# baldhat/yolov10-3D

Measured on AMD Instinct MI355X. Metric: train_images_per_sec, higher is better.
Workload: dtype bf16

## Files before the change

### yolov10-3d_amd/csrc/conv_gemm.hip

```cpp
#include "common.h"
#include "conv_frag.h"
#include <cstdlib>

namespace {

struct ConvP {
  const void* x;
  const void* w;
  const float* bias;
  const float* scale;
  const float* shift;
  int act;
  void* y;
  float* part;
  long xsb, xsh, xsw;
  long ysw;
  int B, Hg, Wg;
  int Hq, Wq;
  int Cg, Cn, G;
  int kh, kw, stride, pad;
  int Ktot, Kpad;
  int M;
  int ntx, nty;
};
// ... 531 lines not shown
  long n = (long)Cout * Kpad;
  if (idx >= n) return;
  int k = idx % Kpad;
  int co = idx / Kpad;
  float v = 0.f;
  if (k < taps * Cg_pad) {
    int tap = k / Cg_pad, ci = k - tap * Cg_pad;
    if (ci < Cg) v = w[((long)co * Cg + ci) * taps + tap];
  }
  TT<T>::st(out + idx, v);
}

template <typename T>
__global__ void pack_w_dgrad_kernel(const float* __restrict__ w, T* __restrict__ out, int G, int Cn, int Cg, int taps, int Kpad) {
  long idx = (long)blockIdx.x * blockDim.x + threadIdx.x;
  long n = (long)G * Cg * Kpad;
  if (idx >= n) return;
  int k = idx % Kpad;
  int ci = (idx / Kpad) % Cg;
  int g = idx / ((long)Kpad * Cg);
  float v = 0.f;
  if (k < taps * Cn) {
    int tap = k / Cn, co = k - tap * Cn;
    v = w[((long)(g * Cn + co) * Cg + ci) * taps + tap];
  }
  TT<T>::st(out + idx, v);
}

template <typename T>
__global__ __launch_bounds__(256) void mt_pack_w_kernel(const long* __restrict__ desc, const int* __restrict__ ctensor, const int* __restrict__ coff,
                                                        int chunk) {
  constexpr int CAP = 4096;
  __shared__ float st[CAP + 64];
  const long* d = desc + (long)ctensor[blockIdx.x] * 8;
  const float* __restrict__ w = (const float*)d[0];
  T* __restrict__ out = (T*)d[1];
  const int a = (int)d[2], b = (int)d[3], c = (int)d[4], taps = (int)d[5], Kpad = (int)d[6], mode = (int)d[7];
  const long n = mode == 0 ? (long)a * Kpad : (long)a * c * Kpad;
  const long beg = (long)coff[blockIdx.x] * chunk;
  const long end = beg + chunk < n ? beg + chunk : n;
  const int tid = threadIdx.x;
  const long rb = beg / Kpad, re = (end - 1) / Kpad;
  if (mode == 0) {
    for (long idx = beg + tid; idx < end; idx += 256) {
      const int k = (int)(idx % Kpad), co = (int)(idx / Kpad);
      float v = 0.f;
      if (k < taps * c) {
        const int tap = k / c, ci = k - tap * c;
        if (ci < b) v = w[((long)co * b + ci) * taps + tap];
      }
      TT<T>::st(out + idx, v);
    }
  } else {
    const int CB = b < 256 ? b : 256;
    int R = CAP / (taps * (CB + 1));
    if (R < 1) R = 1;
    const int P = CB + 1;
    for (long r0 = rb; r0 <= re;) {
      const int g = (int)(r0 / c), ci0 = (int)(r0 - (long)g * c);
      int nr = R;
      if (nr > c - ci0) nr = c - ci0;
      if (nr > re - r0 + 1) nr = (int)(re - r0 + 1);
      const int seg = nr * taps;
      for (int co0 = 0; co0 < b; co0 += CB) {
        const int cb = b - co0 < CB ? b - co0 : CB;
        __syncthreads();
        for (int i = tid; i < cb * seg; i += 256) {
          const int col = i / seg, j = i - col * seg;
          st[j * P + col] = w[((long)(g * b + co0 + col) * c + ci0) * taps + j];
        }
        __syncthreads();
        for (int o = tid; o < seg * cb; o += 256) {
          const int j = o / cb, col = o - j * cb;
          const int cil = j / taps, tap = j - cil * taps;
          const long idx = (r0 + cil) * Kpad + (long)tap * b + co0 + col;
          if (idx >= beg && idx < end) TT<T>::st(out + idx, st[j * P + col]);
        }
      }
      for (int o = tid; o < nr * (Kpad - taps * b); o += 256) {
        const int rl = o / (Kpad - taps * b), k = taps * b + o - rl * (Kpad - taps * b);
        const long idx = (r0 + rl) * Kpad + k;
        if (idx >= beg && idx < end) TT<T>::st(out + idx, 0.f);
      }
      r0 += nr;
    }
  }
}

template <typename T, int MODE>
int launch_conv_mode(ConvP p, hipStream_t st) {
  dim3 block(256);
  const unsigned ny = MODE == 2 ? 4 : 1;
  p.ntx = MODE == 2 ? cdiv((long)p.B * ((p.Hq + 1) / 2) * ((p.Wq + 1) / 2), 128) : cdiv(p.M, 128);
  const long t128 = (long)p.ntx * cdiv(p.Cn, 128) * ny * p.G;
  int bc = p.Cn > 64 ? 128 : (p.Cn > 32 ? 64 : 32);
  if (p.Cn % 32 == 0) {
    if (bc == 128 && t128 < 192) bc = 64;
    if (bc == 64 && (long)p.ntx * cdiv(p.Cn, 64) * ny * p.G < 192 && p.Cn > 32) bc = 32;
  }
  p.nty = cdiv(p.Cn, bc);
  if (bc == 128) {
    size_t sm = 2 * (128 + 128) * 128;
    hipLaunchKernelGGL((conv_gemm_kernel<T, 128, 128, 2, 2, MODE>), dim3(p.ntx * p.nty, ny, p.G), block, sm, st, p);
  } else if (bc == 64) {
    size_t sm = 2 * (128 + 64) * 128;
    hipLaunchKernelGGL((conv_gemm_kernel<T, 128, 64, 4, 1, MODE>), dim3(p.ntx * p.nty, ny, p.G), block, sm, st, p);
  } else {
    size_t sm = 2 * (128 + 32) * 128;
    hipLaunchKernelGGL((conv_gemm_kernel<T, 128, 32, 4, 1, MODE>), dim3(p.ntx * p.nty, ny, p.G), block, sm, st, p);
  }
  Y3D_LAUNCH_CHECK();
  return Y3D_OK;
}

template <typename T, bool DGRAD>
int launch_conv(ConvP p, hipStream_t st) {
  if (DGRAD && p.kh == 3 && p.kw == 3 && p.stride == 2 && p.pad == 1 && p.Cg % TT<T>::CE == 0) return launch_conv_mode<T, 2>(p, st);
  return launch_conv_mode<T, DGRAD ? 1 : 0>(p, st);
}

}

int y3d_conv3x3_tile_route(int dtype, int B, int H, int W, int Cg, int Cn, int G, int kh, int kw, int stride, int pad);
int y3d_conv3x3_flat_tiles(int B, int H, int W);
int y3d_conv3x3_tile_launch(int dtype, int route, const void* x, long xsb, long xsh, long xsw, int B, int H, int W, int Cg, int Cn, int G,
                            const void* w, int Ktot, void* y, long ysw, float* part, int flip, const float* scale, const float* shift, int act,
                            void* stream);

int y3d_wgrad_tile_height(int dtype, int H, int W, int Cg, int Cn, int kh, int kw, int stride, int pad);
int y3d_wgrad_tile_splits(int th, int B, int H, int W, int Cg, int Cn, int G);
int y3d_conv3x3_wgrad_tile_launch(int th, const void* x, long xsb, long xsh, long xsw, const void* dy, long dsw, int B, int H, int W, int Cg,
                                  int Cn, int G, float* slab, int nsplit, void* stream);

int y3d_conv1x1_stream_ok(int dtype, long M, int K, int N, long xsw, int G = 1);
int y3d_conv1x1_stream_launch(const void* x, long xsw, const void* w, int Kpad, const float* bias, const float* scale, const float* shift, int act,
                              void* y, long ysw, float* part, long M, int K, int N, int G, void* stream);
int y3d_wgrad1x1_stream_ok(int dtype, long M, int Cg, int Cn, long xsw, long dsw);
int y3d_wgrad1x1_stream_launch(const void* x, long xsw, const void* dy, long dsw, long M, int Cg, int Cn, float* slab, int nsplit, int chunk_px,
                               void* stream);
int y3d_conv3x3s2_dgrad_ok(int dtype, int B, int Ho, int Wo, int H, int W, int Cout, int Cin, long dsw, long xsw);
int y3d_conv3x3s2_dgrad_launch(const void* dy, long dsw, int B, int Ho, int Wo, int Cout, const void* w_packed_dgrad, int Kpad, void* dx, long xsw,
                               int H, int W, int Cin, void* stream);
int y3d_conv3x3_small_ok(int dtype, int B, int H, int W, int Cin, int Cout, int rows);
int y3d_conv3x3_small_launch(const void* x, long xsb, long xsh, long xsw, int B, int H, int W, int Cin, int Cout, const void* w, int Ktot, void* y,
                             long ysw, float* part, int rows, int flip, const float* scale, const float* shift, int act, const void* res, long rsw,
                             void* stream);
int y3d_conv3x3_small_rows(int B, int H, int W, int Cin, int Cout);
int y3d_conv3x3_small_s2_ok(int dtype, int B, int H, int W, int Cin, int Cout);
int y3d_conv3x3_small_s2_rows(int B, int H, int W, int Cin, int Cout);
int y3d_conv3x3_small_s2_launch(const void* x, long xsb, long xsh, long xsw, int B, int H, int W, int Cin, int Cout, const void* w, int Ktot, void* y,
                                long ysw, float* part, int rows, const float* scale, const float* shift, int act, void* stream);
int y3d_conv1x1_stream_rows(long M, int K, int N, int G = 1);
int y3d_wgrad3x3_small_ok(int dtype, int B, int H, int W, int Cin, int Cout);
int y3d_wgrad3x3_small_splits(int B, int H, int W);
int y3d_wgrad3x3_small_launch(const void* x, long xsb, long xsh, long xsw, const void* dy, long dsw, int B, int H, int W, int Cin, int Cout,
                              float* slab, int nsplit, void* stream);
static inline bool dense_pixels(int B, int H, int W, long sb, long sh, long sw) {
  return (H == 1 || sh == (long)W * sw) && (B == 1 || sb == (long)H * W * sw);
}

static int g_tile_kernels = 1;
extern "C" int y3d_conv2d_wgrad_splits(int dtype, int B, int Ho, int Wo, int Cout, int Cin_g, int groups, int kh, int kw);

static int conv_route(int dtype, int op, int epi, int B, int H, int W, int Ho, int Wo, int Cin, int Cout, int groups, int kh, int kw, int stride,
                      int pad, bool dense, long asw, long bsw, bool cin_full) {
  const int ce = dtype == Y3D_BF16 ? 8 : 4;
  const bool k1 = kh == 1 && kw == 1 && stride == 1 && pad == 0, k3s1 = kh == 3 && kw == 3 && stride == 1 && pad == 1,
             k3s2 = kh == 3 && kw == 3 && stride == 2 && pad == 1;
  if (op == Y3D_OP_FWD) {
    Y3D_CHECK(dtype == Y3D_BF16 || dtype == Y3D_F32, "conv2d_fwd: bad dtype %d", dtype);
    Y3D_CHECK(B > 0 && H > 0 && W > 0 && Cin > 0 && Cout > 0 && groups > 0, "conv2d_fwd: empty shape");
    Y3D_CHECK(Cin % groups == 0 && Cout % groups == 0, "conv2d_fwd: channels not divisible by groups");
    Y3D_CHECK((Cin / groups) % ce == 0, "conv2d_fwd: Cin/groups=%d must be a multiple of %d (pad the input)", Cin / groups, ce);
    Y3D_CHECK(kh * kw <= 64, "conv2d_fwd: at most 64 filter taps");
    Y3D_CHECK(epi >= Y3D_EPI_RAW && epi <= Y3D_EPI_BIAS, "conv2d_fwd: bad epilogue %d", epi);
    const int Cg = Cin / groups, Cn = Cout / groups;
    const long M = (long)B * Ho * Wo;
    const bool bias = epi == Y3D_EPI_BIAS;
    if (k1 && dense && y3d_conv1x1_stream_ok(dtype, M, Cg, Cn, asw, groups)) return Y3D_ROUTE_STREAM1X1;
    Y3D_CHECK(!(epi == Y3D_EPI_PARTIALS && k1 && y3d_conv1x1_stream_ok(dtype, M, Cg, Cn, Cin, groups)),
              "conv2d_fwd: 1x1 input view must be pixel-dense and below 4 GB for the BatchNorm partial layout of this shape");
    if (k3s1 && groups == 1 && !bias && y3d_conv3x3_small_ok(dtype, B, H, W, Cin, Cout, 1)) return Y3D_ROUTE_SMALL;
    Y3D_CHECK(epi != Y3D_EPI_AFFINE_RES, "conv2d_fwd_affine_res: no kernel with a residual epilogue takes this geometry (ask y3d_conv2d_fwd_affine_res_ok first)");
    if (k3s2 && groups == 1 && !bias && y3d_conv3x3_small_s2_ok(dtype, B, H, W, Cin, Cout)) return Y3D_ROUTE_SMALL_S2;
    if (!bias && g_tile_kernels) return y3d_conv3x3_tile_route(dtype, B, H, W, Cg, Cn, groups, kh, kw, stride, pad);
    return Y3D_ROUTE_GENERIC;
  }
  if (op == Y3D_OP_BWD_DATA) {
    Y3D_CHECK(dtype == Y3D_BF16 || dtype == Y3D_F32, "conv2d_bwd_data: bad dtype %d", dtype);
    Y3D_CHECK(groups > 0 && Cin % groups == 0 && Cout % groups == 0, "conv2d_bwd_data: channels not divisible by groups");
    Y3D_CHECK((Cout / groups) % ce == 0, "conv2d_bwd_data: Cout/groups=%d must be a multiple of %d", Cout / groups, ce);
    Y3D_CHECK(kh * kw <= 64, "conv2d_bwd_data: at most 64 filter taps");
    Y3D_CHECK(epi == 0, "conv2d_bwd_data: no epilogue variants");
    const int Cg = Cout / groups, Cn = Cin / groups;
    if (k1 && dense && y3d_conv1x1_stream_ok(dtype, (long)B * H * W, Cg, Cn, asw, groups)) return Y3D_ROUTE_STREAM1X1;
    if (k3s1 && groups == 1 && Ho == H && Wo == W && y3d_conv3x3_small_ok(dtype, B, H, W, Cout, Cin, 1)) return Y3D_ROUTE_SMALL;
    if (k3s2 && groups == 1 && dense && y3d_conv3x3s2_dgrad_ok(dtype, B, Ho, Wo, H, W, Cout, Cin, asw, bsw)) return Y3D_ROUTE_S2_DGRAD;
    if (g_tile_kernels && Ho == H && Wo == W) return y3d_conv3x3_tile_route(dtype, B, H, W, Cg, Cn, groups, kh, kw, stride, pad);
    return Y3D_ROUTE_GENERIC;
  }
  Y3D_CHECK(op == Y3D_OP_BWD_WEIGHT, "conv2d_route: bad op %d", op);
  Y3D_CHECK(dtype == Y3D_BF16 || dtype == Y3D_F32, "conv2d_bwd_weight: bad dtype %d", dtype);
  Y3D_CHECK(groups > 0 && Cin % groups == 0 && Cout % groups == 0, "conv2d_bwd_weight: channels not divisible by groups");
  Y3D_CHECK((Cin / groups) % ce == 0 && (Cout / groups) % ce == 0, "conv2d_bwd_weight: per-group channels must be multiples of %d", ce);
  Y3D_CHECK(epi == 0, "conv2d_bwd_weight: no epilogue variants");
  if (k3s1 && groups == 1 && cin_full && y3d_wgrad3x3_small_ok(dtype, B, H, W, Cin, Cout)) return Y3D_ROUTE_WGRAD_SMALL;
  if (g_tile_kernels && cin_full && y3d_wgrad_tile_height(dtype, H, W, Cin / groups, Cout / groups, kh, kw, stride, pad)) return Y3D_ROUTE_WGRAD_TILE;
  if (k1 && groups == 1 && cin_full && dense && y3d_wgrad1x1_stream_ok(dtype, (long)B * Ho * Wo, Cin, Cout, asw, bsw)) return Y3D_ROUTE_WGRAD_STREAM1X1;
  return Y3D_ROUTE_GENERIC;
}

extern "C" {

int y3d_get_tile_kernels(void) { return g_tile_kernels; }

int y3d_set_tile_kernels(int enable) {
  int old = g_tile_kernels;
  g_tile_kernels = enable ? 1 : 0;
  return old;
}

int y3d_conv_stat_blocks(int B, int Ho, int Wo) { return cdiv((long)B * Ho * Wo, 128); }

int y3d_conv2d_route(int dtype, int op, int epi, int B, int H, int W, int Cin, int Cout, int groups, int kh, int kw, int stride, int pad) {
  Y3D_CHECK(kh > 0 && kw > 0 && stride > 0 && pad >= 0, "conv2d_route: bad filter geometry");
  const int Ho = (H + 2 * pad - kh) / stride + 1, Wo = (W + 2 * pad - kw) / stride + 1;
  Y3D_CHECK(Ho > 0 && Wo > 0, "conv2d_route: empty output");
  if (op == Y3D_OP_BWD_DATA) return conv_route(dtype, op, epi, B, H, W, Ho, Wo, Cin, Cout, groups, kh, kw, stride, pad, true, Cout, Cin, true);
  return conv_route(dtype, op, epi, B, H, W, Ho, Wo, Cin, Cout, groups, kh, kw, stride, pad, true, Cin, Cout, true);
}

int y3d_conv2d_wgrad_plan(int dtype, int B, int H, int W, int Cin, int Cout, int groups, int kh, int kw, int stride, int pad) {
  int Ho = (H + 2 * pad - kh) / stride + 1, Wo = (W + 2 * pad - kw) / stride + 1;
  switch (conv_route(dtype, Y3D_OP_BWD_WEIGHT, 0, B, H, W, Ho, Wo, Cin, Cout, groups, kh, kw, stride, pad, true, Cin, Cout, true)) {
    case Y3D_ROUTE_WGRAD_SMALL: return y3d_wgrad3x3_small_splits(B, H, W);
    case Y3D_ROUTE_WGRAD_TILE:
      return y3d_wgrad_tile_splits(y3d_wgrad_tile_height(dtype, H, W, Cin / groups, Cout / groups, kh, kw, stride, pad), B, H, W, Cin / groups,
                                   Cout / groups, groups);
    case Y3D_ROUTE_WGRAD_STREAM1X1: {
      const int target = 256;
      const long tiles = (long)cdiv(Cin, Cin <= 64 ? 64 : 128) * cdiv(Cout, Cout <= 64 ? 64 : 128);
      long want = target / tiles, maxs = cdiv((long)B * H * W, 4 * 64);
      if (want > maxs) want = maxs;
      return (int)(want < 1 ? 1 : want);
    }
    default: return y3d_conv2d_wgrad_splits(dtype, B, Ho, Wo, Cout, Cin / groups, groups, kh, kw);
  }
}

int y3d_conv2d_stat_rows(int dtype, int B, int H, int W, int Cin, int Cout, int groups, int kh, int kw, int stride, int pad) {
  int Ho = (H + 2 * pad - kh) / stride + 1, Wo = (W + 2 * pad - kw) / stride + 1;
  switch (conv_route(dtype, Y3D_OP_FWD, Y3D_EPI_PARTIALS, B, H, W, Ho, Wo, Cin, Cout, groups, kh, kw, stride, pad, true, Cin, Cout, true)) {
    case Y3D_ROUTE_STREAM1X1: return y3d_conv1x1_stream_rows((long)B * H * W, Cin / groups, Cout / groups, groups);
    case Y3D_ROUTE_SMALL: return y3d_conv3x3_small_rows(B, H, W, Cin, Cout);
    case Y3D_ROUTE_SMALL_S2: return y3d_conv3x3_small_s2_rows(B, H, W, Cin, Cout);
    case Y3D_ROUTE_FLAT: return y3d_conv3x3_flat_tiles(B, H, W);
    case Y3D_ROUTE_TILE8: case Y3D_ROUTE_WIDE3_8: return B * cdiv(H, 8) * cdiv(W, 16);
    case Y3D_ROUTE_TILE16: case Y3D_ROUTE_WIDE3_16: return B * cdiv(H, 16) * cdiv(W, 16);
    default: return cdiv((long)B * Ho * Wo, 128);
  }
}

int y3d_conv_kpad(int dtype, int k_total) {
  int ce = dtype == Y3D_BF16 ? 8 : 4;
  return cdiv(k_total, ce) * ce;
}

int y3d_pack_weight_fwd(int dtype, const float* w_oihw, void* out, int Cout, int Cin_g, int Cin_g_pad, int kh, int kw, void* stream) {
  int ce = dtype == Y3D_BF16 ? 8 : 4;
  Y3D_CHECK(Cin_g_pad >= Cin_g && Cin_g_pad % ce == 0, "pack_weight_fwd: Cin_g_pad=%d must be a multiple of %d", Cin_g_pad, ce);
  int taps = kh * kw, Kpad = taps * Cin_g_pad;
  long n = (long)Cout * Kpad;
  hipStream_t st = (hipStream_t)stream;
  if (dtype == Y3D_BF16)
    hipLaunchKernelGGL(pack_w_fwd_kernel<bf16_t>, dim3(cdiv(n, 256)), dim3(256), 0, st, w_oihw, (bf16_t*)out, Cout, Cin_g, Cin_g_pad, taps, Kpad);
  else
    hipLaunchKernelGGL(pack_w_fwd_kernel<float>, dim3(cdiv(n, 256)), dim3(256), 0, st, w_oihw, (float*)out, Cout, Cin_g, Cin_g_pad, taps, Kpad);
  Y3D_LAUNCH_CHECK();
  return Y3D_OK;
}

int y3d_pack_weight_dgrad(int dtype, const float* w_oihw, void* out, int Cout, int Cin_g, int groups, int kh, int kw, void* stream) {
  Y3D_CHECK(Cout % groups == 0, "pack_weight_dgrad: Cout %% groups");
  int Cn = Cout / groups, taps = kh * kw;
  int Kpad = y3d_conv_kpad(dtype, taps * Cn);
  long n = (long)groups * Cin_g * Kpad;
  hipStream_t st = (hipStream_t)stream;
  if (dtype == Y3D_BF16)
    hipLaunchKernelGGL(pack_w_dgrad_kernel<bf16_t>, dim3(cdiv(n, 256)), dim3(256), 0, st, w_oihw, (bf16_t*)out, groups, Cn, Cin_g, taps, Kpad);
  else
    hipLaunchKernelGGL(pack_w_dgrad_kernel<float>, dim3(cdiv(n, 256)), dim3(256), 0, st, w_oihw, (float*)out, groups, Cn, Cin_g, taps, Kpad);
  Y3D_LAUNCH_CHECK();
  return Y3D_OK;
}

static int check_align(const char* what, const void* ptr, long s0, long s1, long s2, int ce) {
  Y3D_CHECK(((uintptr_t)ptr & 15) == 0, "%s: pointer not 16-byte aligned", what);
  Y3D_CHECK(s0 % ce == 0 && s1 % ce == 0 && s2 % ce == 0, "%s: strides (%ld,%ld,%ld) not multiples of %d elements", what, s0, s1, s2, ce);
  return Y3D_OK;
}

static int conv2d_fwd_impl(int dtype, const void* x, int64_t xsb, int64_t xsh, int64_t xsw, int B, int H, int W, int Cin,
                           const void* w_packed, const float* bias, const float* scale, const float* shift, int act, void* y, int64_t ysw,
                           int Ho, int Wo, int Cout, int groups, int kh, int kw, int stride, int pad, float* stat_partials, void* stream,
                           const void* res = nullptr, int64_t rsw = 0) {
  int ce = dtype == Y3D_BF16 ? 8 : 4;
  Y3D_CHECK(!(bias && stat_partials), "conv2d_fwd: bias and BN partials are mutually exclusive");
  const int epi = res ? Y3D_EPI_AFFINE_RES : scale ? Y3D_EPI_AFFINE : stat_partials ? Y3D_EPI_PARTIALS : bias ? Y3D_EPI_BIAS : Y3D_EPI_RAW;
  const int route = conv_route(dtype, Y3D_OP_FWD, epi, B, H, W, Ho, Wo, Cin, Cout, groups, kh, kw, stride, pad, dense_pixels(B, H, W, xsb, xsh, xsw),
                               xsw, 0, true);
  if (route < 0) return route;
  Y3D_CHECK(Ho == (H + 2 * pad - kh) / stride + 1 && Wo == (W + 2 * pad - kw) / stride + 1, "conv2d_fwd: output dims (%d,%d) inconsistent", Ho, Wo);
  Y3D_CHECK(ysw >= Cout, "conv2d_fwd: ysw < Cout");
  if (check_align("conv2d_fwd x", x, xsb, xsh, xsw, ce)) return Y3D_ERR_INVALID;
  Y3D_CHECK(((uintptr_t)w_packed & 15) == 0 && ((uintptr_t)y & 7) == 0, "conv2d_fwd: w/y alignment");
  Y3D_CHECK((long)B * Ho * Wo < (1L << 31), "conv2d_fwd: too many pixels");
  ConvP p;
  p.x = x; p.w = w_packed; p.bias = bias; p.scale = scale; p.shift = shift; p.act = act; p.y = y; p.part = stat_partials;
  p.xsb = xsb; p.xsh = xsh; p.xsw = xsw; p.ysw = ysw;
  p.B = B; p.Hg = H; p.Wg = W; p.Hq = Ho; p.Wq = Wo;
  p.Cg = Cin / groups; p.Cn = Cout / groups; p.G = groups;
  p.kh = kh; p.kw = kw; p.stride = stride; p.pad = pad;
  p.Ktot = kh * kw * p.Cg; p.Kpad = p.Ktot; p.M = B * Ho * Wo;
  switch (route) {
    case Y3D_ROUTE_STREAM1X1:
      return y3d_conv1x1_stream_launch(x, xsw, w_packed, p.Kpad, bias, scale, shift, act, y, ysw, stat_partials, p.M, p.Cg, p.Cn, groups, stream);
    case Y3D_ROUTE_SMALL: {
      const int rows = stat_partials ? y3d_conv3x3_small_rows(B, H, W, Cin, Cout) : 1;
      return y3d_conv3x3_small_launch(x, xsb, xsh, xsw, B, H, W, Cin, Cout, w_packed, p.Ktot, y, ysw, stat_partials, rows, 0, scale, shift, act, res, rsw, stream);
    }
    case Y3D_ROUTE_SMALL_S2: {
      const int rows = stat_partials ? y3d_conv3x3_small_s2_rows(B, H, W, Cin, Cout) : 1;
      return y3d_conv3x3_small_s2_launch(x, xsb, xsh, xsw, B, H, W, Cin, Cout, w_packed, p.Ktot, y, ysw, stat_partials, rows, scale, shift, act, stream);
    }
    case Y3D_ROUTE_GENERIC:
      if (dtype == Y3D_BF16) return launch_conv<bf16_t, false>(p, (hipStream_t)stream);
      return launch_conv<float, false>(p, (hipStream_t)stream);
    default:
      return y3d_conv3x3_tile_launch(dtype, route, x, xsb, xsh, xsw, B, H, W, p.Cg, p.Cn, groups, w_packed, p.Ktot, y, ysw, stat_partials, 0, scale,
                                     shift, act, stream);
  }
}

int y3d_conv2d_fwd(int dtype, const void* x, int64_t xsb, int64_t xsh, int64_t xsw, int B, int H, int W, int Cin,
                   const void* w_packed, const float* bias, void* y, int64_t ysw, int Ho, int Wo, int Cout, int groups,
                   int kh, int kw, int stride, int pad, float* stat_partials, void* stream) {
  return conv2d_fwd_impl(dtype, x, xsb, xsh, xsw, B, H, W, Cin, w_packed, bias, nullptr, nullptr, 0, y, ysw, Ho, Wo, Cout, groups, kh, kw,
                         stride, pad, stat_partials, stream);
}

int y3d_conv2d_fwd_affine(int dtype, const void* x, int64_t xsb, int64_t xsh, int64_t xsw, int B, int H, int W, int Cin,
                          const void* w_packed, const float* scale, const float* shift, int act, void* y, int64_t ysw, int Ho, int Wo,
                          int Cout, int groups, int kh, int kw, int stride, int pad, void* stream) {
  Y3D_CHECK(scale && shift, "conv2d_fwd_affine: scale/shift required");
  return conv2d_fwd_impl(dtype, x, xsb, xsh, xsw, B, H, W, Cin, w_packed, nullptr, scale, shift, act, y, ysw, Ho, Wo, Cout, groups, kh, kw,
                         stride, pad, nullptr, stream);
}

int y3d_conv2d_fwd_affine_res_ok(int dtype, int B, int H, int W, int Cin, int Cout, int groups, int kh, int kw, int stride, int pad) {
  return kh == 3 && kw == 3 && stride == 1 && pad == 1 && groups == 1 && y3d_conv3x3_small_ok(dtype, B, H, W, Cin, Cout, 1);
}

int y3d_conv2d_fwd_affine_res(int dtype, const void* x, int64_t xsb, int64_t xsh, int64_t xsw, int B, int H, int W, int Cin,
                              const void* w_packed, const float* scale, const float* shift, int act, const void* res, int64_t rsw, void* y,
                              int64_t ysw, int Ho, int Wo, int Cout, int groups, int kh, int kw, int stride, int pad, void* stream) {
  Y3D_CHECK(scale && shift && res, "conv2d_fwd_affine_res: scale / shift / residual required");
  Y3D_CHECK(y3d_conv2d_fwd_affine_res_ok(dtype, B, H, W, Cin, Cout, groups, kh, kw, stride, pad), "conv2d_fwd_affine_res: geometry not supported");
  return conv2d_fwd_impl(dtype, x, xsb, xsh, xsw, B, H, W, Cin, w_packed, nullptr, scale, shift, act, y, ysw, Ho, Wo, Cout, groups, kh, kw,
                         stride, pad, nullptr, stream, res, rsw);
}

int y3d_conv2d_bwd_data(int dtype, const void* dy, int64_t dsb, int64_t dsh, int64_t dsw, int B, int Ho, int Wo, int Cout,
                        const void* w_packed_dgrad, void* dx, int64_t xsw, int H, int W, int Cin, int groups, int kh, int kw,
                        int stride, int pad, void* stream) {
  int ce = dtype == Y3D_BF16 ? 8 : 4;
  const int route = conv_route(dtype, Y3D_OP_BWD_DATA, 0, B, H, W, Ho, Wo, Cin, Cout, groups, kh, kw, stride, pad,
                               dense_pixels(B, Ho, Wo, dsb, dsh, dsw), dsw, xsw, true);
  if (route < 0) return route;
  Y3D_CHECK(xsw >= Cin, "conv2d_bwd_data: xsw < Cin");
  Y3D_CHECK(stride >= 1 && dsh % stride == 0 && dsw % stride == 0, "conv2d_bwd_data: stride %d must divide the dy strides", stride);
  if (check_align("conv2d_bwd_data dy", dy, dsb, dsh, dsw, ce)) return Y3D_ERR_INVALID;
  ConvP p;
  p.x = dy; p.w = w_packed_dgrad; p.bias = nullptr; p.scale = nullptr; p.shift = nullptr; p.act = 0; p.y = dx; p.part = nullptr;
  p.xsb = dsb; p.xsh = dsh; p.xsw = dsw; p.ysw = xsw;
  p.B = B; p.Hg = Ho; p.Wg = Wo; p.Hq = H; p.Wq = W;
  p.Cg = Cout / groups; p.Cn = Cin / groups; p.G = groups;
  p.kh = kh; p.kw = kw; p.stride = stride; p.pad = pad;
  p.Ktot = kh * kw * p.Cg; p.Kpad = y3d_conv_kpad(dtype, p.Ktot); p.M = B * H * W;
// ... 111 lines not shown
```

### yolov10-3d_amd/csrc/wgrad3x3_small.hip

```cpp
#include "common.h"
#include <type_traits>

namespace {

struct WsP {
  const bf16_t* x;
  const bf16_t* dy;
  float* slab;
  int xsb, xsh, xsw, dsw;
  int B, H, W, Cout, Cin;
  int nty, ntx, ntiles;
  unsigned xbytes, dbytes;
};

template <int OFF>
__device__ __forceinline__ s16x4_t ws_tr(unsigned a) {
  s16x4_t v;
  asm volatile("ds_read_b64_tr_b16 %0, %1 offset:%2" : "=v"(v) : "v"(a), "n"(OFF));
  return v;
}
template <int N, int CT>
__device__ __forceinline__ void ws_wait(s16x4_t (&b)[3][2], s16x4_t (&a)[CT][2]) {
  if constexpr (CT == 1)
    asm volatile("s_waitcnt lgkmcnt(%8)" : "+v"(b[0][0]), "+v"(b[0][1]), "+v"(b[1][0]), "+v"(b[1][1]), "+v"(b[2][0]), "+v"(b[2][1]), "+v"(a[0][0]), "+v"(a[0][1]) : "n"(N));
  else if constexpr (CT == 2)
    asm volatile("s_waitcnt lgkmcnt(%10)" : "+v"(b[0][0]), "+v"(b[0][1]), "+v"(b[1][0]), "+v"(b[1][1]), "+v"(b[2][0]), "+v"(b[2][1]), "+v"(a[0][0]), "+v"(a[0][1]),
                 "+v"(a[1][0]), "+v"(a[1][1]) : "n"(N));
  else if constexpr (CT == 3)
    asm volatile("s_waitcnt lgkmcnt(%12)" : "+v"(b[0][0]), "+v"(b[0][1]), "+v"(b[1][0]), "+v"(b[1][1]), "+v"(b[2][0]), "+v"(b[2][1]), "+v"(a[0][0]), "+v"(a[0][1]),
                 "+v"(a[1][0]), "+v"(a[1][1]), "+v"(a[2][0]), "+v"(a[2][1]) : "n"(N));
  else {
    static_assert(CT == 4, "1..4 output-channel tiles per wave");
    asm volatile("s_waitcnt lgkmcnt(%14)" : "+v"(b[0][0]), "+v"(b[0][1]), "+v"(b[1][0]), "+v"(b[1][1]), "+v"(b[2][0]), "+v"(b[2][1]), "+v"(a[0][0]), "+v"(a[0][1]),
                 "+v"(a[1][0]), "+v"(a[1][1]), "+v"(a[2][0]), "+v"(a[2][1]), "+v"(a[3][0]), "+v"(a[3][1]) : "n"(N));
  }
}

template <int CB, int NCT>
__global__ __launch_bounds__(256) void wgrad3x3_small_kernel(WsP p) {
  constexpr int CIN = CB / 2, NCIT = CIN / 16;
  constexpr int WCI = NCIT >= 4 ? 4 : NCIT;
  constexpr int WCO = 4 / WCI;
  constexpr int CT = NCT / WCO;
  static_assert(NCT % WCO == 0 && CT >= 1 && CT <= 4, "output-channel tiles must split over the waves");
  constexpr int HW = 18, NPIX = 10 * HW;
  constexpr int CPD = NCT * 2 + 2, PD = CPD * 16;
  constexpr int CPX = CB / 16 + 2, PX = CPX * 16;
  constexpr int ID = 2 * CPD;
  constexpr int IX = (NPIX * CPX + 63) / 64;
  constexpr int NI = (ID + IX + 3) / 4;
  constexpr int DBY = ID * 1024, BUF = (ID + IX) * 1024;
  constexpr int NBUF = 3;
  extern __shared__ __attribute__((aligned(16))) char smem[];
  const int tid = threadIdx.x, lane = tid & 63, wave = __builtin_amdgcn_readfirstlane(tid >> 6);
  const int wci = wave % WCI, wco = wave / WCI;
  const int nwk = gridDim.x, wk = blockIdx.x;
  const __amdgpu_buffer_rsrc_t rd = __builtin_amdgcn_make_buffer_rsrc((void*)p.dy, 0, (int)p.dbytes, 0x00020000);
  const __amdgpu_buffer_rsrc_t rx = __builtin_amdgcn_make_buffer_rsrc((void*)p.x, 0, (int)p.xbytes, 0x00020000);
  constexpr unsigned OOB = 0xfffffff0u;
  const unsigned sbase = (unsigned)(size_t)(__attribute__((address_space(3))) const char*)smem;
  auto decode = [&](int t, int& b, int& y0, int& x0) {
    const int tx = t % p.ntx, t2 = t / p.ntx;
    x0 = tx * 16;
    y0 = (t2 % p.nty) * 8;
    b = t2 / p.nty;
  };
  int p_off[NI], p_rc[NI];
#pragma unroll
  for (int n = 0; n < NI; ++n) {
    const int gi = wave * NI + n;
    if (gi < ID) {
      const int q = gi * 64 + lane, m = q / CPD, col = q - m * CPD;
      const bool ok = (col < NCT * 2) & (col * 8 < p.Cout);
      p_off[n] = ((m >> 4) * p.W + (m & 15)) * p.dsw + col * 8;
      p_rc[n] = ((ok ? (m >> 4) : 255) << 8) | (m & 15);
    } else {
      const int q = (gi - ID) * 64 + lane, P = q / CPX, col = q - P * CPX;
      const int hr = P / HW, hc = P - hr * HW;
      const bool ok = (gi < ID + IX) & (P < NPIX) & (col < CB / 16) & (col * 8 < p.Cin);
      p_off[n] = (hr - 1) * p.xsh + (hc - 1) * p.xsw + col * 8;
      p_rc[n] = ((ok ? hr : 255) << 8) | hc;
    }
  }
  auto issue = [&](int t, int buf) {
    int b, y0, x0;
    const bool live = t < p.ntiles;
    decode(live ? t : 0, b, y0, x0);
    const int baseD = ((b * p.H + y0) * p.W + x0) * p.dsw, baseX = b * p.xsb + y0 * p.xsh + x0 * p.xsw;
    const int hlim = live ? p.H : 0;
#pragma unroll
    for (int n = 0; n < NI; ++n) {
      const int r = p_rc[n] >> 8, c = p_rc[n] & 255;
      const int gi = wave * NI + n;
      if (gi < ID) {
        const bool ok = (y0 + r < hlim) & (x0 + c < p.W);
        __builtin_amdgcn_raw_ptr_buffer_load_lds(rd, (__attribute__((address_space(3))) void*)(size_t)(sbase + buf * BUF + gi * 1024), 16,
                                                 ok ? (unsigned)(baseD + p_off[n]) * 2u : OOB, 0, 0, 0);
      } else {
        const bool ok = ((unsigned)(y0 - 1 + r) < (unsigned)hlim) & ((unsigned)(x0 - 1 + c) < (unsigned)p.W);
        const unsigned dst = gi < ID + IX ? sbase + buf * BUF + gi * 1024 : sbase + NBUF * BUF;
        __builtin_amdgcn_raw_ptr_buffer_load_lds(rx, (__attribute__((address_space(3))) void*)(size_t)dst, 16, ok ? (unsigned)(baseX + p_off[n]) * 2u : OOB, 0, 0, 0);
      }
    }
  };
  issue(wk, 0);
  issue(wk + nwk, 1);

  f32x4_t acc[9][CT];
#pragma unroll
  for (int t = 0; t < 9; ++t)
#pragma unroll
    for (int a = 0; a < CT; ++a) acc[t][a] = (f32x4_t){0.f, 0.f, 0.f, 0.f};
  const int g = lane >> 4, li = lane & 15;
  const unsigned offA = (4 * g + (li >> 2)) * PD + (wco * CT * 16 + 4 * (li & 3)) * 2;
  const unsigned offB = DBY + (4 * g + (li >> 2)) * PX + (wci * 16 + 4 * (li & 3)) * 2;
  int buf = 0;
#pragma unroll 1
  for (int t = wk; t < p.ntiles; t += nwk) {
    asm volatile("s_waitcnt vmcnt(%0)" ::"n"(NI) : "memory");
    __builtin_amdgcn_s_barrier();
    issue(t + 2 * nwk, buf >= 1 ? buf - 1 : NBUF - 1);
    const unsigned tb = sbase + buf * BUF;
    const unsigned aA = tb + offA, aB = tb + offB;
    s16x4_t fb[2][3][2], fa[2][CT][2];
    auto reads = [&](auto KS, auto R, auto SETC) {
      constexpr int ks = decltype(KS)::value, r = decltype(R)::value, set = decltype(SETC)::value;
      if constexpr (r == 0) {
        constexpr int kb = ks & 1;
        fa[kb][0][0] = ws_tr<(32 * ks) * PD>(aA);
        fa[kb][0][1] = ws_tr<(32 * ks + 16) * PD>(aA);
        if constexpr (CT > 1) { fa[kb][1][0] = ws_tr<(32 * ks) * PD + 32>(aA); fa[kb][1][1] = ws_tr<(32 * ks + 16) * PD + 32>(aA); }
        if constexpr (CT > 2) { fa[kb][2][0] = ws_tr<(32 * ks) * PD + 64>(aA); fa[kb][2][1] = ws_tr<(32 * ks + 16) * PD + 64>(aA); }
        if constexpr (CT > 3) { fa[kb][3][0] = ws_tr<(32 * ks) * PD + 96>(aA); fa[kb][3][1] = ws_tr<(32 * ks + 16) * PD + 96>(aA); }
      }
      fb[set][0][0] = ws_tr<((2 * ks + r) * HW + 0) * PX>(aB);
      fb[set][0][1] = ws_tr<((2 * ks + 1 + r) * HW + 0) * PX>(aB);
      fb[set][1][0] = ws_tr<((2 * ks + r) * HW + 1) * PX>(aB);
      fb[set][1][1] = ws_tr<((2 * ks + 1 + r) * HW + 1) * PX>(aB);
      fb[set][2][0] = ws_tr<((2 * ks + r) * HW + 2) * PX>(aB);
      fb[set][2][1] = ws_tr<((2 * ks + 1 + r) * HW + 2) * PX>(aB);
    };
    auto mfmas = [&](auto KS, auto R, auto SETC) {
      constexpr int ks = decltype(KS)::value, r = decltype(R)::value, set = decltype(SETC)::value;
      typedef __attribute__((ext_vector_type(8))) short s16x8_t;
#pragma unroll
      for (int q = 0; q < 3; ++q) {
        const bf16x8_t b = __builtin_bit_cast(bf16x8_t, (s16x8_t)__builtin_shufflevector(fb[set][q][0], fb[set][q][1], 0, 1, 2, 3, 4, 5, 6, 7));
#pragma unroll
        for (int a = 0; a < CT; ++a) {
          const bf16x8_t av = __builtin_bit_cast(bf16x8_t, (s16x8_t)__builtin_shufflevector(fa[ks & 1][a][0], fa[ks & 1][a][1], 0, 1, 2, 3, 4, 5, 6, 7));
          acc[r * 3 + q][a] = __builtin_amdgcn_mfma_f32_16x16x32_bf16(av, b, acc[r * 3 + q][a], 0, 0, 0);
        }
      }
    };
#define WS_I(n) std::integral_constant<int, n>()
#define WS_STEP(KS, R, NKS, NR, SET, NEXTN)                                     \
    reads(WS_I(NKS), WS_I(NR), WS_I((SET) ^ 1));                                \
    ws_wait<NEXTN, CT>(fb[SET], fa[(KS) & 1]);                                  \
    mfmas(WS_I(KS), WS_I(R), WS_I(SET));
    reads(WS_I(0), WS_I(0), WS_I(0));
    WS_STEP(0, 0, 0, 1, 0, 6) WS_STEP(0, 1, 0, 2, 1, 6) WS_STEP(0, 2, 1, 0, 0, 6 + 2 * CT)
    WS_STEP(1, 0, 1, 1, 1, 6) WS_STEP(1, 1, 1, 2, 0, 6) WS_STEP(1, 2, 2, 0, 1, 6 + 2 * CT)
    WS_STEP(2, 0, 2, 1, 0, 6) WS_STEP(2, 1, 2, 2, 1, 6) WS_STEP(2, 2, 3, 0, 0, 6 + 2 * CT)
    WS_STEP(3, 0, 3, 1, 1, 6) WS_STEP(3, 1, 3, 2, 0, 6)
    ws_wait<0, CT>(fb[1], fa[1]);
    mfmas(WS_I(3), WS_I(2), WS_I(1));
#undef WS_STEP
#undef WS_I
    if (++buf == NBUF) buf = 0;
  }
  asm volatile("s_waitcnt vmcnt(0)" ::: "memory");
  const int cin = p.Cin;
  float* slab = p.slab + (long)wk * p.Cout * (9 * cin);
#pragma unroll
  for (int t = 0; t < 9; ++t)
#pragma unroll
    for (int a = 0; a < CT; ++a)
#pragma unroll
      for (int r = 0; r < 4; ++r) {
        const int co = (wco * CT + a) * 16 + 4 * g + r;
        if (co < p.Cout && wci * 16 + li < cin) slab[(long)co * (9 * cin) + t * cin + wci * 16 + li] = acc[t][a][r];
      }
}

template <int CB, int NCT>
void ws_launch(const WsP& p, int grid, hipStream_t st) {
  constexpr int CPD = NCT * 2 + 2, CPX = CB / 16 + 2, ID = 2 * CPD, IX = (180 * CPX + 63) / 64;
  const size_t lds = (size_t)3 * (ID + IX) * 1024 + 1024;
  static bool attr = false;
  if (!attr) {
    (void)hipFuncSetAttribute((const void*)wgrad3x3_small_kernel<CB, NCT>, hipFuncAttributeMaxDynamicSharedMemorySize, 160 * 1024);
    attr = true;
  }
  hipLaunchKernelGGL((wgrad3x3_small_kernel<CB, NCT>), dim3(grid), dim3(256), lds, st, p);
}

}

extern "C" int y3d_get_stream1x1(void);

int y3d_wgrad3x3_small_ok(int dtype, int B, int H, int W, int Cin, int Cout) {
  if (!y3d_get_stream1x1() || dtype != Y3D_BF16 || (Cin != 32 && (Cin <= 32 || Cin > 64 || Cin % 8 != 0)) || Cout % 16 != 0 || Cout < 16 || Cout > 64) return 0;
  if (Cin == 32 && (Cout / 16) % 2 != 0) return 0;
  if (H < 4 || W < 8) return 0;
  return 1;
}

int y3d_wgrad3x3_small_splits(int B, int H, int W) {
  const long ntiles = (long)B * cdiv(H, 8) * cdiv(W, 16);
  return (int)(ntiles < 256 ? ntiles : 256);
}

int y3d_wgrad3x3_small_launch(const void* x, long xsb, long xsh, long xsw, const void* dy, long dsw, int B, int H, int W, int Cin, int Cout,
                              float* slab, int nsplit, void* stream) {
  Y3D_CHECK(((uintptr_t)x & 15) == 0 && xsb % 8 == 0 && xsh % 8 == 0 && xsw % 8 == 0 && ((uintptr_t)dy & 15) == 0 && dsw % 8 == 0,
            "wgrad3x3_small: operand alignment");
  Y3D_CHECK(nsplit == y3d_wgrad3x3_small_splits(B, H, W), "wgrad3x3_small: nsplit must come from y3d_conv2d_wgrad_plan");
  const long xext = ((long)(B - 1) * xsb + (long)(H - 1) * xsh + (long)(W - 1) * xsw + Cin) * 2;
  const long dext = (((long)B * H * W - 1) * dsw + Cout) * 2;
  Y3D_CHECK(xext < (1L << 32) - 64 && dext < (1L << 32) - 64 && (long)B * xsb < (1L << 31) && (long)B * H * W * dsw < (1L << 31),
            "wgrad3x3_small: tensors beyond 32-bit byte offsets");
  WsP p;
  p.x = (const bf16_t*)x; p.dy = (const bf16_t*)dy; p.slab = slab;
  p.xsb = (int)xsb; p.xsh = (int)xsh; p.xsw = (int)xsw; p.dsw = (int)dsw;
  p.B = B; p.H = H; p.W = W; p.Cout = Cout; p.Cin = Cin;
  p.nty = cdiv(H, 8); p.ntx = cdiv(W, 16); p.ntiles = B * p.nty * p.ntx;
  p.xbytes = (unsigned)xext; p.dbytes = (unsigned)dext;
  hipStream_t st = (hipStream_t)stream;
  const int nct = Cout / 16;
  if (Cin > 32) {
    switch (nct) {
      case 1: ws_launch<128, 1>(p, nsplit, st); break;
      case 2: ws_launch<128, 2>(p, nsplit, st); break;
      case 3: ws_launch<128, 3>(p, nsplit, st); break;
      default: ws_launch<128, 4>(p, nsplit, st); break;
    }
  } else {
    if (nct == 2) ws_launch<64, 2>(p, nsplit, st); else ws_launch<64, 4>(p, nsplit, st);
  }
  Y3D_LAUNCH_CHECK();
  return Y3D_OK;
}
```

Before: 1425.

## Extend small 3x3 wgrad kernel to 128-channel layers via channel-block grid

The small-tile 3x3 weight-gradient kernel now splits larger channel counts (64/128 in and out) into 64x64 channel blocks along a second grid dimension, offsetting loads and slab writes per block. The split count is divided by the number of channel blocks so the total block count stays bounded. The 64-out-channel, wide-input variant now runs with 8 waves per block instead of 4. This routes mid-sized 3x3 layers away from the generic tiled wgrad path, but it re-reads inputs once per channel block and changes register and LDS pressure for the 8-wave variant.

Result: no change. 1424, median of 3 (-0.1%).

```diff
diff --git a/yolov10-3d_amd/csrc/conv_gemm.hip b/yolov10-3d_amd/csrc/conv_gemm.hip
--- a/yolov10-3d_amd/csrc/conv_gemm.hip
+++ b/yolov10-3d_amd/csrc/conv_gemm.hip
@@ -707,7 +707,7 @@
                                 long ysw, float* part, int rows, const float* scale, const float* shift, int act, void* stream);
 int y3d_conv1x1_stream_rows(long M, int K, int N, int G = 1);
 int y3d_wgrad3x3_small_ok(int dtype, int B, int H, int W, int Cin, int Cout);
-int y3d_wgrad3x3_small_splits(int B, int H, int W);
+int y3d_wgrad3x3_small_splits(int B, int H, int W, int Cin, int Cout);
 int y3d_wgrad3x3_small_launch(const void* x, long xsb, long xsh, long xsw, const void* dy, long dsw, int B, int H, int W, int Cin, int Cout,
                               float* slab, int nsplit, void* stream);
 static inline bool dense_pixels(int B, int H, int W, long sb, long sh, long sw) {
@@ -788,7 +788,7 @@
 int y3d_conv2d_wgrad_plan(int dtype, int B, int H, int W, int Cin, int Cout, int groups, int kh, int kw, int stride, int pad) {
   int Ho = (H + 2 * pad - kh) / stride + 1, Wo = (W + 2 * pad - kw) / stride + 1;
   switch (conv_route(dtype, Y3D_OP_BWD_WEIGHT, 0, B, H, W, Ho, Wo, Cin, Cout, groups, kh, kw, stride, pad, true, Cin, Cout, true)) {
-    case Y3D_ROUTE_WGRAD_SMALL: return y3d_wgrad3x3_small_splits(B, H, W);
+    case Y3D_ROUTE_WGRAD_SMALL: return y3d_wgrad3x3_small_splits(B, H, W, Cin, Cout);
     case Y3D_ROUTE_WGRAD_TILE:
       return y3d_wgrad_tile_splits(y3d_wgrad_tile_height(dtype, H, W, Cin / groups, Cout / groups, kh, kw, stride, pad), B, H, W, Cin / groups,
                                    Cout / groups, groups);
diff --git a/yolov10-3d_amd/csrc/wgrad3x3_small.hip b/yolov10-3d_amd/csrc/wgrad3x3_small.hip
--- a/yolov10-3d_amd/csrc/wgrad3x3_small.hip
+++ b/yolov10-3d_amd/csrc/wgrad3x3_small.hip
@@ -9,6 +9,7 @@
   float* slab;
   int xsb, xsh, xsw, dsw;
   int B, H, W, Cout, Cin;
+  int Cout_all, Cin_all;
   int nty, ntx, ntiles;
   unsigned xbytes, dbytes;
 };
@@ -36,11 +37,11 @@
   }
 }
 
-template <int CB, int NCT>
-__global__ __launch_bounds__(256) void wgrad3x3_small_kernel(WsP p) {
+template <int CB, int NCT, int NW>
+__global__ __launch_bounds__(NW * 64) void wgrad3x3_small_kernel(WsP p) {
   constexpr int CIN = CB / 2, NCIT = CIN / 16;
   constexpr int WCI = NCIT >= 4 ? 4 : NCIT;
-  constexpr int WCO = 4 / WCI;
+  constexpr int WCO = NW / WCI;
   constexpr int CT = NCT / WCO;
   static_assert(NCT % WCO == 0 && CT >= 1 && CT <= 4, "output-channel tiles must split over the waves");
   constexpr int HW = 18, NPIX = 10 * HW;
@@ -48,13 +49,14 @@
   constexpr int CPX = CB / 16 + 2, PX = CPX * 16;
   constexpr int ID = 2 * CPD;
   constexpr int IX = (NPIX * CPX + 63) / 64;
-  constexpr int NI = (ID + IX + 3) / 4;
+  constexpr int NI = (ID + IX + NW - 1) / NW;
   constexpr int DBY = ID * 1024, BUF = (ID + IX) * 1024;
   constexpr int NBUF = 3;
   extern __shared__ __attribute__((aligned(16))) char smem[];
   const int tid = threadIdx.x, lane = tid & 63, wave = __builtin_amdgcn_readfirstlane(tid >> 6);
   const int wci = wave % WCI, wco = wave / WCI;
   const int nwk = gridDim.x, wk = blockIdx.x;
+  const int nbi = p.Cin_all / p.Cin, ci0 = (blockIdx.y % nbi) * p.Cin, co0 = (blockIdx.y / nbi) * p.Cout;
   const __amdgpu_buffer_rsrc_t rd = __builtin_amdgcn_make_buffer_rsrc((void*)p.dy, 0, (int)p.dbytes, 0x00020000);
   const __amdgpu_buffer_rsrc_t rx = __builtin_amdgcn_make_buffer_rsrc((void*)p.x, 0, (int)p.xbytes, 0x00020000);
   constexpr unsigned OOB = 0xfffffff0u;
@@ -72,13 +74,13 @@
     if (gi < ID) {
       const int q = gi * 64 + lane, m = q / CPD, col = q - m * CPD;
       const bool ok = (col < NCT * 2) & (col * 8 < p.Cout);
-      p_off[n] = ((m >> 4) * p.W + (m & 15)) * p.dsw + col * 8;
+      p_off[n] = ((m >> 4) * p.W + (m & 15)) * p.dsw + co0 + col * 8;
       p_rc[n] = ((ok ? (m >> 4) : 255) << 8) | (m & 15);
     } else {
       const int q = (gi - ID) * 64 + lane, P = q / CPX, col = q - P * CPX;
       const int hr = P / HW, hc = P - hr * HW;
       const bool ok = (gi < ID + IX) & (P < NPIX) & (col < CB / 16) & (col * 8 < p.Cin);
-      p_off[n] = (hr - 1) * p.xsh + (hc - 1) * p.xsw + col * 8;
+      p_off[n] = (hr - 1) * p.xsh + (hc - 1) * p.xsw + ci0 + col * 8;
       p_rc[n] = ((ok ? hr : 255) << 8) | hc;
     }
   }
@@ -170,8 +172,8 @@
     if (++buf == NBUF) buf = 0;
   }
   asm volatile("s_waitcnt vmcnt(0)" ::: "memory");
-  const int cin = p.Cin;
-  float* slab = p.slab + (long)wk * p.Cout * (9 * cin);
+  const int cin = p.Cin_all;
+  float* slab = p.slab + (long)wk * p.Cout_all * (9 * cin) + (long)co0 * (9 * cin) + ci0;
 #pragma unroll
   for (int t = 0; t < 9; ++t)
 #pragma unroll
@@ -179,64 +181,80 @@
 #pragma unroll
       for (int r = 0; r < 4; ++r) {
         const int co = (wco * CT + a) * 16 + 4 * g + r;
-        if (co < p.Cout && wci * 16 + li < cin) slab[(long)co * (9 * cin) + t * cin + wci * 16 + li] = acc[t][a][r];
-      }
-}
-
-template <int CB, int NCT>
-void ws_launch(const WsP& p, int grid, hipStream_t st) {
+        if (co < p.Cout && wci * 16 + li < p.Cin) slab[(long)co * (9 * cin) + t * cin + wci * 16 + li] = acc[t][a][r];
+      }
+}
+
+template <int CB, int NCT, int NW = 4>
+void ws_launch(const WsP& p, dim3 grid, hipStream_t st) {
   constexpr int CPD = NCT * 2 + 2, CPX = CB / 16 + 2, ID = 2 * CPD, IX = (180 * CPX + 63) / 64;
   const size_t lds = (size_t)3 * (ID + IX) * 1024 + 1024;
   static bool attr = false;
   if (!attr) {
-    (void)hipFuncSetAttribute((const void*)wgrad3x3_small_kernel<CB, NCT>, hipFuncAttributeMaxDynamicSharedMemorySize, 160 * 1024);
+    (void)hipFuncSetAttribute((const void*)wgrad3x3_small_kernel<CB, NCT, NW>, hipFuncAttributeMaxDynamicSharedMemorySize, 160 * 1024);
     attr = true;
   }
-  hipLaunchKernelGGL((wgrad3x3_small_kernel<CB, NCT>), dim3(grid), dim3(256), lds, st, p);
+  hipLaunchKernelGGL((wgrad3x3_small_kernel<CB, NCT, NW>), dim3(grid), dim3(NW * 64), lds, st, p);
 }
 
 }
 
 extern "C" int y3d_get_stream1x1(void);
 
+static void ws_blocks(int Cin, int Cout, int& cib, int& cob) {
+  cib = Cin > 64 ? 64 : Cin;
+  cob = Cout > 64 ? 64 : Cout;
+}
+
 int y3d_wgrad3x3_small_ok(int dtype, int B, int H, int W, int Cin, int Cout) {
-  if (!y3d_get_stream1x1() || dtype != Y3D_BF16 || (Cin != 32 && (Cin <= 32 || Cin > 64 || Cin % 8 != 0)) || Cout % 16 != 0 || Cout < 16 || Cout > 64) return 0;
+  if (!y3d_get_stream1x1() || dtype != Y3D_BF16 || H < 4 || W < 8) return 0;
+  if (Cin > 64 || Cout > 64) {
+    return (Cin == 64 || Cin == 128) && (Cout == 64 || Cout == 128) && H >= 32 && W >= 32 && H <= 64 && W <= 64;
+  }
+  if ((Cin != 32 && (Cin <= 32 || Cin % 8 != 0)) || Cout % 16 != 0 || Cout < 16) return 0;
   if (Cin == 32 && (Cout / 16) % 2 != 0) return 0;
-  if (H < 4 || W < 8) return 0;
   return 1;
 }
 
-int y3d_wgrad3x3_small_splits(int B, int H, int W) {
+int y3d_wgrad3x3_small_splits(int B, int H, int W, int Cin, int Cout) {
   const long ntiles = (long)B * cdiv(H, 8) * cdiv(W, 16);
-  return (int)(ntiles < 256 ? ntiles : 256);
+  int cib, cob;
+  ws_blocks(Cin, Cout, cib, cob);
+  const int nblk = (Cin / cib) * (Cout / cob);
+  const long want = 256 / nblk;
+  return (int)(ntiles < want ? ntiles : want);
 }
 
 int y3d_wgrad3x3_small_launch(const void* x, long xsb, long xsh, long xsw, const void* dy, long dsw, int B, int H, int W, int Cin, int Cout,
                               float* slab, int nsplit, void* stream) {
   Y3D_CHECK(((uintptr_t)x & 15) == 0 && xsb % 8 == 0 && xsh % 8 == 0 && xsw % 8 == 0 && ((uintptr_t)dy & 15) == 0 && dsw % 8 == 0,
             "wgrad3x3_small: operand alignment");
-  Y3D_CHECK(nsplit == y3d_wgrad3x3_small_splits(B, H, W), "wgrad3x3_small: nsplit must come from y3d_conv2d_wgrad_plan");
+  Y3D_CHECK(nsplit == y3d_wgrad3x3_small_splits(B, H, W, Cin, Cout), "wgrad3x3_small: nsplit must come from y3d_conv2d_wgrad_plan");
+  Y3D_CHECK(xsw >= Cin && dsw >= Cout, "wgrad3x3_small: pixel strides below the channel counts");
   const long xext = ((long)(B - 1) * xsb + (long)(H - 1) * xsh + (long)(W - 1) * xsw + Cin) * 2;
   const long dext = (((long)B * H * W - 1) * dsw + Cout) * 2;
   Y3D_CHECK(xext < (1L << 32) - 64 && dext < (1L << 32) - 64 && (long)B * xsb < (1L << 31) && (long)B * H * W * dsw < (1L << 31),
             "wgrad3x3_small: tensors beyond 32-bit byte offsets");
+  int cib, cob;
+  ws_blocks(Cin, Cout, cib, cob);
   WsP p;
   p.x = (const bf16_t*)x; p.dy = (const bf16_t*)dy; p.slab = slab;
   p.xsb = (int)xsb; p.xsh = (int)xsh; p.xsw = (int)xsw; p.dsw = (int)dsw;
-  p.B = B; p.H = H; p.W = W; p.Cout = Cout; p.Cin = Cin;
+  p.B = B; p.H = H; p.W = W; p.Cout = cob; p.Cin = cib; p.Cout_all = Cout; p.Cin_all = Cin;
   p.nty = cdiv(H, 8); p.ntx = cdiv(W, 16); p.ntiles = B * p.nty * p.ntx;
   p.xbytes = (unsigned)xext; p.dbytes = (unsigned)dext;
   hipStream_t st = (hipStream_t)stream;
-  const int nct = Cout / 16;
-  if (Cin > 32) {
+  const dim3 grid(nsplit, (Cin / cib) * (Cout / cob));
+  const int nct = cob / 16;
+  if (cib > 32) {
     switch (nct) {
-      case 1: ws_launch<128, 1>(p, nsplit, st); break;
-      case 2: ws_launch<128, 2>(p, nsplit, st); break;
-      case 3: ws_launch<128, 3>(p, nsplit, st); break;
-      default: ws_launch<128, 4>(p, nsplit, st); break;
+      case 1: ws_launch<128, 1>(p, grid, st); break;
+      case 2: ws_launch<128, 2>(p, grid, st); break;
+      case 3: ws_launch<128, 3>(p, grid, st); break;
+      default: ws_launch<128, 4, 8>(p, grid, st); break;
     }
   } else {
-    if (nct == 2) ws_launch<64, 2>(p, nsplit, st); else ws_launch<64, 4>(p, nsplit, st);
+    if (nct == 2) ws_launch<64, 2>(p, grid, st); else ws_launch<64, 4>(p, grid, st);
   }
   Y3D_LAUNCH_CHECK();
   return Y3D_OK;
```
